# wuer5/OMGSR

Measured on AMD Instinct MI355X. Metric: SR images/sec, higher is better.
Workload: dtype fp16; 1 GPU; OMGSR-S 256->1024, batch=4/GPU, accurate tier (fp32 stream, fp16 MFMA operands + split corrections), tiled VAE 256/64; global_batch=4, latent_tile=64, tile_overlap=32, world_size=1, parallelism=dp1, weights=seeded random, SD2.1-base shapes

## Files before the change

omgsr_amd/csrc/igemm.hip:

```cpp
#include "common.hip.h"
#include "../../include/omgsr_hip.h"
#include "timing.hip.h"
#include "igemm_epilogue.hip.h"
#include "igemm_launch.hip.h"
#include <stdlib.h>
#include <stdio.h>
#include <string.h>

namespace omgsr { static int g_batch_invariant = 0; }
extern "C" int omgsr_set_batch_invariant(int on) { omgsr::g_batch_invariant = (on != 0); return 0; }

namespace {

omgsr_igemm_args policy_view(const omgsr_igemm_args& a) {
    omgsr_igemm_args p = a;
    if (omgsr::g_batch_invariant && a.batch == 1) {
        const int64_t howo = (int64_t)a.Ho * a.Wo;
        const int64_t rows = a.sample_rows > 0 ? a.sample_rows : howo;
        if (rows >= howo) p.N = (int32_t)(rows / howo);
        else { p.N = 1; p.Ho = 1; p.Wo = (int32_t)rows; }
        if (p.N < 1) p.N = 1;
    }
    return p;
}
// ... 369 lines not shown
    }
    if (a.workspace && splitk_plan(a, M64) > 1) return;
    if (omgsr::g_batch_invariant) return;
    const int howo = a.Ho * a.Wo;
    if (howo % 32) return;
    *nslot = howo / 32;
    *entries = (pow2 && gsz <= 32) ? a.gn_groups : a.Cout;
}
}

namespace {
bool gn_fusable(const omgsr_igemm_args& a_in) {
    static const char* off = getenv("OMGSR_GN_FUSE");
    if (off && off[0] == '0') return false;
    omgsr_igemm_args a = a_in;
    a.gn_scale_shift = nullptr;
    if (!omgsr::igemm_halo_gn_geometry_ok(a) || a.out_layout != OMGSR_LAYOUT_NHWC || a.act == OMGSR_ACT_GEGLU) return false;
    if ((int64_t)a.H * a.W * a.Cin >= (1ll << 31)) return false;
    if (a.workspace && splitk_plan(a, (int64_t)a.N * a.Ho * a.Wo) > 1) return false;
    if (!use_halo(a) || use_halo_phase(a)) return false;
    if (omgsr::igemm_halo_flat(a) != 0) return false;
    static const char* mc = getenv("OMGSR_GN_FUSE_MAX_COUT");
    static const int max_cout = mc ? atoi(mc) : 128;
    const int logical_cols = (a.act == OMGSR_ACT_GEGLU) ? 2 * a.Cout : a.Cout;
    return logical_cols <= max_cout;
}
}

extern "C" int32_t omgsr_igemm_gn_fusable(const omgsr_igemm_args* ap) { return (ap && gn_fusable(*ap)) ? 1 : 0; }
extern "C" int32_t omgsr_igemm_out_mx6_ok(const omgsr_igemm_args* ap) {
    if (!ap) return 0;
    omgsr_igemm_args a = *ap;
    a.out_mx = 6;
    return out_mx6_ok(a) ? 1 : 0;
}

extern "C" int32_t omgsr_igemm_gn_slots(const omgsr_igemm_args* ap) {
    if (!ap) return 0;
    int nslot, entries;
    gn_plan(*ap, &nslot, &entries);
    return nslot;
}

extern "C" int32_t omgsr_igemm_gn_entries(const omgsr_igemm_args* ap) {
    if (!ap) return 0;
    int nslot, entries;
    gn_plan(*ap, &nslot, &entries);
    return entries;
}

extern "C" int64_t omgsr_igemm_workspace_bytes(const omgsr_igemm_args* ap) {
    if (!ap || ap->mxf8) return 0;
    const int64_t M64 = (int64_t)ap->N * ap->Ho * ap->Wo;
    const int splits = splitk_plan(*ap, M64);
    if (splits < 2) return 0;
    const int logical_cols = (ap->act == OMGSR_ACT_GEGLU) ? 2 * ap->Cout : ap->Cout;
    return (int64_t)splits * M64 * (((logical_cols + 127) / 128) * 128) * 4;
}

namespace {
int validate_args(omgsr_igemm_args& a) {
    if (!a.in || !a.weight || !a.out) return OMGSR_E_BADARG;
    if (a.N <= 0 || a.H <= 0 || a.W <= 0 || a.Cin <= 0 || a.Cout <= 0 || a.Ho <= 0 || a.Wo <= 0 ||
        a.R <= 0 || a.S <= 0 || a.stride <= 0 || a.batch <= 0) return OMGSR_E_BADARG;
    if ((a.Cin & 7) || (a.Cout_pad & 127) || (a.K_pad % BK) || a.K_pad < a.R * a.S * a.Cin) return OMGSR_E_SHAPE;
    if (a.upsample != 0 && a.upsample != 1) return OMGSR_E_BADARG;
    const int64_t M64 = (int64_t)a.N * a.Ho * a.Wo;
    if (M64 >= (1ll << 31)) return OMGSR_E_SHAPE;
    const int logical_cols = (a.act == OMGSR_ACT_GEGLU) ? 2 * a.Cout : a.Cout;
    if (logical_cols > a.Cout_pad) return OMGSR_E_SHAPE;
    if (a.act == OMGSR_ACT_GEGLU && ((a.Cout & 31) || a.out_layout != OMGSR_LAYOUT_NHWC)) return OMGSR_E_SHAPE;
    if (a.out_layout == OMGSR_LAYOUT_T && (a.t_rows <= 0 || a.t_ld < a.t_rows || a.residual)) return OMGSR_E_BADARG;
    if (a.out_ld != 0 && (a.out_ld < a.Cout || a.out_layout != OMGSR_LAYOUT_NHWC)) return OMGSR_E_BADARG;
    if (a.res_el != OMGSR_EL_16 && a.res_el != OMGSR_EL_F32) return OMGSR_E_BADARG;
    if (a.res_el == OMGSR_EL_F32 && a.residual && a.act == OMGSR_ACT_GEGLU) return OMGSR_E_SHAPE;
    if (a.out_lo_off < 0) return OMGSR_E_BADARG;
    if (a.out_lo_off && (a.out_dtype != OMGSR_OUT_BF16 || a.out_layout != OMGSR_LAYOUT_NHWC || (a.Cout & 7) || (a.out_ld & 7) || (a.out_lo_off & 7) ||
                         a.out_lo_off < a.Cout || a.out_ld < a.out_lo_off + a.Cout || a.gn_partial)) return OMGSR_E_SHAPE;
    if (a.in_split && ((a.in_ld > 0 ? a.in_ld : a.Cin) & 15)) return OMGSR_E_SHAPE;
    if (a.in_ld < 0 || (a.in_ld & 7) || (a.in_ld > 0 && (a.in_ld > a.Cin || a.Cin > 2 * a.in_ld))) return OMGSR_E_SHAPE;
    if (a.in_ld == a.Cin) a.in_ld = 0;
    const int ksegs = 1 + (a.in_split ? 1 : 0) + (a.w_split ? 1 : 0);
    if (a.Cin % (8 * ksegs)) return OMGSR_E_SHAPE;
    if (a.mx_chunks16 < 0 || (a.mx_chunks16 > 0 && !mx_geometry_ok(a) && !omgsr::igemm_gmx_ok(a))) return OMGSR_E_SHAPE;
    if (a.mx_chunks16 > 0 && a.mx_fmt != 0 && a.mx_fmt != 8 && (a.mx_fmt != 6 || !mx_geometry_ok(a))) return OMGSR_E_SHAPE;
    if (a.out_mx != 0 && a.out_mx != 1 && a.out_mx != 6) return OMGSR_E_BADARG;
    if (a.out_mx == 6 && !out_mx6_ok(a)) return OMGSR_E_SHAPE;
    if (a.out_mx && (a.out_dtype != OMGSR_OUT_BF16 || a.out_layout != OMGSR_LAYOUT_NHWC || (a.Cout & 63) || a.out_lo_off || a.out_ld || a.gn_partial ||
                     omgsr::compute_dtype() != 1)) return OMGSR_E_SHAPE;
    if (a.gn_scale_shift && (a.gn_nimg <= 0 || a.gn_act != OMGSR_ACT_SILU || !gn_fusable(a))) return OMGSR_E_SHAPE;
    if (a.mxf8 != 0 && a.mxf8 != 1) return OMGSR_E_BADARG;
    if (a.mxf8 && !omgsr::mxfp8_gemm_ok(a)) return OMGSR_E_SHAPE;
    if (a.gn_partial) {
        int nslot, entries;
        gn_plan(a, &nslot, &entries);
        if (nslot <= 0 || a.gn_entries != entries) return OMGSR_E_BADARG;
    }
    return 0;
}

void work_of(const omgsr_igemm_args& a, double* flops, double* bytes, const bool out8 = false) {
    const int64_t M64 = (int64_t)a.N * a.Ho * a.Wo;
    const int logical_cols = (a.act == OMGSR_ACT_GEGLU) ? 2 * a.Cout : a.Cout;
    const int ksegs = 1 + (a.in_split ? 1 : 0) + (a.w_split ? 1 : 0);
    *flops = 2.0 * (double)M64 * (double)a.R * a.S * (a.Cin / ksegs) * (double)logical_cols * a.batch;
    const double out_b = out8 ? 1.0 + 1.0 / 32.0 : (a.out_dtype == OMGSR_OUT_F32 ? 4.0 : (a.out_lo_off ? 4.0 : 2.0)), res_b = a.residual ? (a.res_el == OMGSR_EL_F32 ? 4.0 : 2.0) : 0.0;
    const double eb = a.mxf8 ? 1.0 + 1.0 / 32.0 : 2.0;
    *bytes = (eb * ((double)a.N * a.H * a.W * (a.in_ld > 0 ? a.in_ld : a.Cin) + (double)a.Cout_pad * a.K_pad) + (double)M64 * a.Cout * (out_b + res_b)) * a.batch;
}

Geo geo_of(const omgsr_igemm_args& a) {
    Geo g{};
    g.M = (int)((int64_t)a.N * a.Ho * a.Wo);
    g.HoWo = a.Ho * a.Wo;
    g.Hv = a.H << a.upsample;
    g.Wv = a.W << a.upsample;
    g.nk = a.K_pad / BK;
    g.splits = 1; g.nk_total = g.nk;
    return g;
}
}

extern "C" int omgsr_igemm_multi_plan(omgsr_igemm_args* args, int32_t count) {
    if (!args || count <= 0) return OMGSR_E_BADARG;
    static const char* off = getenv("OMGSR_MULTI");
    int total = 0, total_ph = 0, total_flat = 0;
    bool all_flat_ok = true;
    for (int i = 0; i < count; ++i) {
        args[i].group_tiles = 0;
        total += omgsr::igemm_halo_tiles_form(args[i], 0);
        total_ph += omgsr::igemm_halo_tiles(args[i], true);
        const int tf = omgsr::igemm_halo_tiles_form(args[i], 1);
        all_flat_ok = all_flat_ok && tf > 0;
        total_flat += tf > 0 ? tf : 0;
    }
    if ((off && off[0] == '0') || omgsr::g_batch_invariant) return 0;
    const bool flat = all_flat_ok && total_flat < total;
    for (int i = 0; i < count; ++i) args[i].group_tiles = (args[i].upsample && args[i].weight_ph) ? total_ph : (flat ? -total_flat : total);
    return 0;
}

extern "C" int omgsr_igemm_multi(const omgsr_igemm_args* args, int32_t count, void* stream) {
    if (!args || count <= 0) return OMGSR_E_BADARG;
    hipStream_t st = (hipStream_t)stream;
    constexpr int MAXG = 8;
    omgsr_igemm_args grp[MAXG];
    Geo geo[MAXG];
    int ng = 0, mode = -1;
    double gf = 0.0, gb = 0.0;
    long long gm = 0;
    auto flush = [&]() -> int {
        if (ng == 0) return 0;
        int rc;
        {
            const int logical_cols = (grp[0].act == OMGSR_ACT_GEGLU) ? 2 * grp[0].Cout : grp[0].Cout;
            omgsr::TimingScope ts(OMGSR_TK_IGEMM, gf, gb, st, gm, logical_cols, (long long)grp[0].R * grp[0].S * grp[0].Cin);
            ts.rec.variant = ng == 1 ? (mode == 1 ? 6 : 3) : (mode == 1 ? 8 : 7);
            if (grp[0].gn_scale_shift) ts.rec.variant = ng == 1 ? 10 : 11;
            if (grp[0].mx_chunks16 > 0 && grp[0].mx_fmt == 6) ts.rec.variant = mode == 1 ? (ng == 1 ? 16 : 17) : (ng == 1 ? 13 : 14);
            rc = ng == 1 ? omgsr::igemm_halo_launch(grp[0], geo[0], st, mode == 1) : omgsr::igemm_halo_launch_multi(grp, geo, ng, st, mode == 1);
        }
        ng = 0; gf = gb = 0.0; gm = 0;
        return rc;
    };
    for (int i = 0; i < count; ++i) {
        omgsr_igemm_args a = args[i];
// ... 366 lines not shown
```

omgsr_amd/csrc/igemm_halo_body.hip.h:

```cpp
#pragma once
#include "common.hip.h"
#include "../../include/omgsr_hip.h"
#include "igemm_epilogue.hip.h"
#include "igemm_launch.hip.h"
#include <stdlib.h>
#include <type_traits>

namespace {

constexpr int TH = 8, TW = 32;
template <int TAPS, bool BIG = false> struct HaloGeo {
    static constexpr int KS = TAPS == 9 ? 3 : 2;
    static constexpr int PW = TW + KS - 1, PH = TH + KS - 1, PROWS = PH * PW;
    static constexpr int APIECES = BIG ? 27 : (PROWS + 15) / 16, APW = (APIECES + 3) / 4;
    static constexpr int A_BYTES = APIECES * 1024;
    static constexpr int NB = TAPS == 9 ? 3 : 4;
    static constexpr int DUMMY_OFF = 2 * A_BYTES, B_OFF = DUMMY_OFF + 2048;
    static constexpr int LDS_BYTES = B_OFF + NB * 128 * 64;
};
constexpr int BN = 128, B_BYTES = BN * 64, BPW = 2;
constexpr int LDS_BYTES = HaloGeo<9>::LDS_BYTES > HaloGeo<4>::LDS_BYTES ? HaloGeo<9>::LDS_BYTES : HaloGeo<4>::LDS_BYTES;
static_assert(HaloGeo<9>::APIECES == 22 && HaloGeo<9>::APW == 6 && HaloGeo<4>::APIECES == 19 && HaloGeo<4>::APW == 5, "piece counts");
constexpr int LDS_BYTES_BIG = HaloGeo<9, true>::LDS_BYTES;
constexpr int GN_MAX_CIN = 1024, LDS_BYTES_GN = HaloGeo<9>::LDS_BYTES + GN_MAX_CIN * 8;
// ... 272 lines not shown
#pragma unroll
                for (int j = 0; j < FN; ++j)
                    asm volatile("s_nop 3\n\tv_mfma_scale_f32_32x32x64_f8f6f4 %0, %1, %2, %0, %3, %4 op_sel_hi:[0,0,0]"
                                 : "+v"(acc[i][j]) : "v"(b8[j]), "v"(a8[i]), "v"(sw), "v"(sa));
                if constexpr (LATE) {
                    if (i == FM / 2 - 1) {
                        __builtin_amdgcn_sched_barrier(0);
                        issue_dma();
                        __builtin_amdgcn_sched_barrier(0);
                    }
                }
            }
            return;
        }
        x8_t<T> af[2][FM], bf[2][FN];
#pragma unroll
        for (int i = 0; i < FM; ++i) {
            af[0][i] = *reinterpret_cast<const x8_t<T>*>(As + i * AIMM + aoff[tap][FLAT ? 0 : i]);
            af[1][i] = *reinterpret_cast<const x8_t<T>*>(As + i * AIMM + (aoff[tap][FLAT ? 0 : i] ^ 32));
        }
#pragma unroll
        for (int j = 0; j < FN; ++j) {
            bf[0][j] = *reinterpret_cast<const x8_t<T>*>(Bs + j * 32 * 64 + boff0);
            bf[1][j] = *reinterpret_cast<const x8_t<T>*>(Bs + j * 32 * 64 + boff1);
        }
        if constexpr (PRIO) __builtin_amdgcn_s_setprio(1);
#pragma unroll
        for (int ks = 0; ks < 2; ++ks) {
#pragma unroll
            for (int i = 0; i < FM; ++i)
#pragma unroll
                for (int j = 0; j < FN; ++j) acc[i][j] = mfma32(bf[ks][j], af[ks][i], acc[i][j]);
            if constexpr (LATE) {
                if (ks == 0) {
                    __builtin_amdgcn_sched_barrier(0);
                    issue_dma();
                    __builtin_amdgcn_sched_barrier(0);
                }
            }
        }
        if constexpr (GNF != 0 && tap >= 2 && tap < 2 + APW) {
            if (cc + 1 < ncc) {
                __builtin_amdgcn_sched_barrier(0);
                u32x4_t g_raw;
                f32x4_t g_tb[4];
                gn_read(tap - 2, par ^ 1, cc + 1, g_raw, g_tb);
                *gn_slot(tap - 2, par ^ 1) = gn_math(tap - 2, g_raw, g_tb);
            }
        }
        if constexpr (PRIO) __builtin_amdgcn_s_setprio(0);
    };
    auto chunk = [&](auto par_c, auto f8_c, const int cc) {
        const int s0 = cc * TAPS;
        step(std::integral_constant<int, 0>{}, par_c, f8_c, cc, s0 + 0);
        step(std::integral_constant<int, 1>{}, par_c, f8_c, cc, s0 + 1);
        step(std::integral_constant<int, 2>{}, par_c, f8_c, cc, s0 + 2);
        step(std::integral_constant<int, 3>{}, par_c, f8_c, cc, s0 + 3);
        if constexpr (TAPS == 9) {
            step(std::integral_constant<int, 4>{}, par_c, f8_c, cc, s0 + 4);
            step(std::integral_constant<int, 5>{}, par_c, f8_c, cc, s0 + 5);
            step(std::integral_constant<int, 6>{}, par_c, f8_c, cc, s0 + 6);
            step(std::integral_constant<int, 7>{}, par_c, f8_c, cc, s0 + 7);
            step(std::integral_constant<int, 8>{}, par_c, f8_c, cc, s0 + 8);
        }
    };
    if (g.main_prio == 1) __builtin_amdgcn_s_setprio(1);
    else if (g.main_prio == 2) __builtin_amdgcn_s_setprio(2);
    int cc = cbeg;
    const int e16 = (SPLITK && n16 > ncc) ? ncc : n16;
    for (; cc < e16; cc += 2) {
        chunk(std::integral_constant<int, 0>{}, std::integral_constant<int, 0>{}, cc);
        if (cc + 1 < e16) chunk(std::integral_constant<int, 1>{}, std::integral_constant<int, 0>{}, cc + 1);
    }
    if constexpr (MX && std::is_same<T, f16_t>::value && !NARROW && ABL == 0 && !PRIO) {
        asm volatile("s_nop 7\n\ts_nop 7" ::: "memory");
        for (; cc < ncc; cc += 2) {
            chunk(std::integral_constant<int, 0>{}, std::integral_constant<int, 1>{}, cc);
            if (cc + 1 < ncc) chunk(std::integral_constant<int, 1>{}, std::integral_constant<int, 1>{}, cc + 1);
        }
        asm volatile("s_nop 15\n\ts_nop 15\n\ts_nop 15\n\ts_nop 15\n\ts_nop 15\n\ts_nop 15" ::: "memory");
    }

    if (g.main_prio) __builtin_amdgcn_s_setprio(0);
    int mb[FM], nv[FM];
    int colsv = (PHASE ? p.W : p.Wo) - x0; colsv = colsv > TW ? TW : colsv;
#pragma unroll
    for (int i = 0; i < FM; ++i) {
        const int y = y0 + FM * wm + i;
        mb[i] = PHASE ? (img * p.Ho + 2 * y + ph_a) * p.Wo + 2 * x0 + ph_b : (img * p.Ho + y) * p.Wo + x0;
        nv[i] = (y < (PHASE ? p.H : p.Ho)) ? colsv : 0;
        if (FP) {
            mb[i] = f0 + TW * (FM * wm + i);
            const int left = p.Ho * FP - mb[i];
            nv[i] = left < 0 ? 0 : (left > TW ? TW : left);
        }
    }
    if constexpr (ABL == 1) { if (p.alpha != 12345.0f) return; }
    {
        float* epi = reinterpret_cast<float*>(lds) + wave * 32 * (WTN + 4);
        const int64_t slot = PHASE ? ((int64_t)(img * per_img + trem) * 2 + wm) * 4 + bidy : (int64_t)(img * per_img + trem) * 2 + wm;
        float* gn_dst = (p.gn_partial && !NARROW) ? p.gn_partial + slot * p.gn_entries * 2 : nullptr;
        igemm_epilogue<T, WTN, FM, FN, OUT6>(p, acc, epi, lane, mb, nv, n0 + wn * WTN, 0, gn_dst, 0, PHASE ? 2 : (FP ? -FP : 1), FP ? img * p.Ho * p.Wo : 0);
    }
}

OMGSR_DEVINL bool phase_block_map(const int b, const int T, const int n8, const bool chunked, int& tile, int& phase) {
    constexpr int CH = 64;
    const int xcd = b & 7, idx = b >> 3;
    int base, cnt;
    if (n8 > 0) { cnt = n8 >> 3; base = xcd * cnt; }
    else {
        const int q = T >> 3, r = T & 7;
        base = xcd < r ? xcd * (q + 1) : r * (q + 1) + (xcd - r) * q;
        cnt = xcd < r ? q + 1 : q;
    }
    if (idx >= 4 * cnt) return false;
    if (chunked) {
        const int chunk = idx / (4 * CH), r = idx - chunk * 4 * CH;
        const int left = cnt - chunk * CH, sz = left < CH ? left : CH;
        phase = r / sz;
        tile = base + chunk * CH + (r - phase * sz);
    } else {
        tile = base + (idx >> 2); phase = idx & 3;
    }
    return tile < T;
}

template <typename T, int ABL, bool PRIO, bool NARROW = false, int TAPS = 9, int MX = 0, int FLAT = 0, int GNF = 0, bool OUT6 = false>
__global__ __launch_bounds__(256, 2) void igemm_halo_kernel(const omgsr_igemm_args p, const IgemmGeo g) {
    int tile, phase;
    if (TAPS == 4 && g.interleave) {
        if (!phase_block_map((int)blockIdx.x, g.ntm * g.ntn, 0, g.interleave == 2, tile, phase)) return;
    } else {
        tile = xcd_remap((int)blockIdx.x, g.ntm * g.ntn); phase = (int)blockIdx.y;
    }
    halo_body<T, ABL, PRIO, NARROW, TAPS, MX, FLAT, GNF, false, OUT6>(p, g, tile, phase);
}

constexpr int HALO_MULTI_MAX = 8;
struct HaloMulti {
    omgsr_igemm_args p[HALO_MULTI_MAX];
    IgemmGeo g[HALO_MULTI_MAX];
    int start[HALO_MULTI_MAX + 1];
    int count;
};
template <typename T, bool NARROW, int TAPS, int MX = 0, int FLAT = 0, int GNF = 0, bool SPLITK = false, bool OUT6 = false>
__global__ __launch_bounds__(256, 2) void igemm_halo_multi_kernel(const HaloMulti m) {
    int s = 0, tile, phase;
    if (TAPS == 4 && m.g[0].interleave) {
        while (s + 1 < m.count && (int)blockIdx.x >= 4 * m.start[s + 1]) ++s;
        if (!phase_block_map((int)blockIdx.x - 4 * m.start[s], m.g[s].ntm * m.g[s].ntn, m.start[s + 1] - m.start[s], m.g[0].interleave == 2, tile, phase)) return;
    } else {
        while (s + 1 < m.count && (int)blockIdx.x >= m.start[s + 1]) ++s;
        const int bid = (int)blockIdx.x - m.start[s];
        if (bid >= m.g[s].ntm * m.g[s].ntn) return;
        tile = xcd_remap(bid, m.g[s].ntm * m.g[s].ntn); phase = (int)blockIdx.y;
    }
    halo_body<T, 0, false, NARROW, TAPS, MX, FLAT, GNF, SPLITK, OUT6>(m.p[s], m.g[s], tile, phase);
}


static inline int halo_flat_eligible(const omgsr_igemm_args& a) {
    static const char* off = getenv("OMGSR_HALO_FLAT");
    if (off && off[0] == '0') return 0;
    if (a.gn_scale_shift) return 0;
    if (a.out_mx == 6) return 0;
    static const char* mw = getenv("OMGSR_HALO_FLAT_MAXW");
    static const int maxw = mw ? atoi(mw) : 80;
    const int logical_cols = (a.act == OMGSR_ACT_GEGLU) ? 2 * a.Cout : a.Cout;
    const int64_t ldo = a.out_ld > 0 ? a.out_ld : a.Cout;
    if (a.R != 3 || a.S != 3 || a.stride != 1 || a.upsample || a.Wo != a.W || a.Ho != a.H || a.Wo > maxw || a.Wo < 4 || logical_cols < 96 || (a.Cout & 7) || (ldo & 7) ||
        a.out_layout != OMGSR_LAYOUT_NHWC || a.act == OMGSR_ACT_GEGLU) return 0;
    return a.Wo + 2;
}
static inline int halo_flat_tiles_per_image(const omgsr_igemm_args& a) { return (a.Ho * (a.Wo + 2) + TH * TW - 1) / (TH * TW); }
static inline int halo_grid_tiles_per_image(const omgsr_igemm_args& a) { return ((a.Wo + TW - 1) / TW) * ((a.Ho + TH - 1) / TH); }
static inline int halo_flat_pitch(const omgsr_igemm_args& a) {
    const int P = halo_flat_eligible(a);
    if (!P) return 0;
    if (a.group_tiles < 0) return P;
    if (a.group_tiles > 0) return 0;
    return halo_flat_tiles_per_image(a) < halo_grid_tiles_per_image(a) ? P : 0;
}

static inline bool halo_geo(const omgsr_igemm_args& a, IgemmGeo& g, const bool phase) {
    const int logical_cols = (a.act == OMGSR_ACT_GEGLU) ? 2 * a.Cout : a.Cout;
    static const char* mp = getenv("OMGSR_HALO_MAINPRIO");
    g.main_prio = mp ? atoi(mp) : 0;
    static const char* il = getenv("OMGSR_PHASE_INTERLEAVE");
    g.interleave = phase ? (il ? atoi(il) : 2) : 0;
    g.nk = a.Cin / 32;
    g.tiles_x = ((phase ? a.W : a.Wo) + TW - 1) / TW;
    g.tiles_y = ((phase ? a.H : a.Ho) + TH - 1) / TH;
    g.flat = phase ? 0 : halo_flat_pitch(a);
    if (g.flat) { g.tiles_x = (a.Ho * g.flat + TH * TW - 1) / (TH * TW); g.tiles_y = 1; }
    g.ntm = a.N * g.tiles_x * g.tiles_y;
    const bool narrow = logical_cols <= 32 && !phase;
    g.ntn = narrow ? 1 : (logical_cols + BN - 1) / BN;
    return narrow;
}

constexpr bool COLS_128 = false, COLS_32 = true;
constexpr int MX_NONE = 0, MX_FP8 = 1, MX_FP6 = 6;
constexpr int FLAT_OFF = 0, FLAT_22 = 1, FLAT_27 = 2;
constexpr int GNF_OFF = 0, GNF_ON = 1;
constexpr bool OUT6_ON = true, SPLITK_ON = true;
constexpr int FLAT_22_MAX_PITCH = 47;

template <typename T, bool NARROW, int TAPS, int MX = MX_NONE, int FLAT = FLAT_OFF, int GNF = GNF_OFF, bool OUT6 = false>
constexpr auto halo_one = &igemm_halo_kernel<T, 0, false, NARROW, TAPS, MX, FLAT, GNF, OUT6>;
template <typename T, bool NARROW, int TAPS, int MX = MX_NONE, int FLAT = FLAT_OFF, int GNF = GNF_OFF, bool OUT6 = false>
constexpr auto halo_group = &igemm_halo_multi_kernel<T, NARROW, TAPS, MX, FLAT, GNF, false, OUT6>;
constexpr int halo_lds_bytes(const int flat, const int gnf) { return gnf ? LDS_BYTES_GN : flat == FLAT_27 ? LDS_BYTES_BIG : LDS_BYTES; }

static inline dim3 halo_grid(const IgemmGeo& g, const bool phase) {
    return (phase && g.interleave) ? dim3(32 * ((g.ntm * g.ntn + 7) / 8)) : dim3(g.ntm * g.ntn, phase ? 4 : 1, 1);
}
static inline dim3 halo_multi_grid(const IgemmGeo& g0, const unsigned blocks, const bool phase) {
    return (phase && g0.interleave) ? dim3(4 * blocks) : dim3(blocks, phase ? 4 : 1, 1);
}

struct HaloPack { int blocks; bool narrow, flat; };
static inline HaloPack halo_multi_pack(const omgsr_igemm_args* a, const IgemmGeo* g0, const int count, const bool phase, HaloMulti& m) {
    HaloPack k{0, false, false};
    m.count = count;
    for (int i = 0; i < count; ++i) {
        m.p[i] = a[i];
        m.g[i] = g0[i];
        const bool narrow = halo_geo(a[i], m.g[i], phase);
        k.narrow = k.narrow || narrow;
        k.flat = k.flat || m.g[i].flat != 0;
        m.start[i] = k.blocks;
        k.blocks += (m.g[i].ntm * m.g[i].ntn + 7) & ~7;
    }
    m.start[count] = k.blocks;
    return k;
}

struct HaloJob {
    const omgsr_igemm_args* a; const IgemmGeo* g;
    const HaloMulti* m; unsigned blocks;
    hipStream_t st;
};
static inline HaloJob halo_job(const omgsr_igemm_args& a, const IgemmGeo& g, hipStream_t st) { return HaloJob{&a, &g, nullptr, 0u, st}; }
static inline HaloJob halo_job(const void* halo_multi, const unsigned blocks, hipStream_t st) {
    return HaloJob{nullptr, nullptr, reinterpret_cast<const HaloMulti*>(halo_multi), blocks, st};
}
template <typename T, bool NARROW, int TAPS, int MX = MX_NONE, int FLAT = FLAT_OFF, int GNF = GNF_OFF, bool OUT6 = false>
int halo_run(const HaloJob& j) {
    constexpr int lds = halo_lds_bytes(FLAT, GNF);
    if (j.m) return launch_lds<halo_group<T, NARROW, TAPS, MX, FLAT, GNF, OUT6>>(halo_multi_grid(j.m->g[0], j.blocks, TAPS == 4), dim3(256), lds, j.st, *j.m);
    return launch_lds<halo_one<T, NARROW, TAPS, MX, FLAT, GNF, OUT6>>(halo_grid(*j.g, TAPS == 4), dim3(256), lds, j.st, *j.a, *j.g);
}
template <int MX>
int halo_mx_run(const HaloJob& j, const bool phase, const bool splitk) {
    if (phase) return halo_run<f16_t, COLS_128, 4, MX>(j);
    if (splitk && !j.m) return OMGSR_E_BADARG;
    if (splitk) return launch_lds<igemm_halo_multi_kernel<f16_t, COLS_128, 9, MX, FLAT_OFF, GNF_OFF, SPLITK_ON>>(halo_multi_grid(j.m->g[0], j.blocks, false), dim3(256), LDS_BYTES, j.st, *j.m);
    return halo_run<f16_t, COLS_128, 9, MX>(j);
}

}
```

omgsr_amd/ops.py:

```python
from __future__ import annotations

import ctypes as C
import os
from contextlib import contextmanager
from dataclasses import dataclass
from typing import NamedTuple, Optional

import torch

from . import _lib
from ._lib import AttnArgs, IgemmArgs, check

ACT_NONE, ACT_SILU, ACT_GELU_TANH, ACT_GEGLU = 0, 1, 2, 3
OUT_STREAM, OUT_BF16, OUT_F32 = -1, 0, 1
LAYOUT_NHWC, LAYOUT_T = 0, 1
EL_16, EL_F32, EL_SPLIT, EL_MX, EL_MX6, EL_MXFP8 = 0, 1, 2, 3, 4, 5
MX_LO_SHIFT = 11


def _el_of_split(split: int) -> int:
    return {1: EL_16, 2: EL_SPLIT, 3: EL_MX, 4: EL_MX6}[split]


_ACT = torch.bfloat16
# ... 151 lines not shown
        raise _lib.OmgsrError(f"{name}: tensor is on {t.device}; the OMGSR HIP path runs on an MI355X only")
    if not t.is_contiguous():
        raise ValueError(f"{name}: must be contiguous")
    return t


def _round_up(x: int, m: int) -> int:
    return (x + m - 1) // m * m


class _GemmGroup:

    def __init__(self):
        self.blocks, self.whats, self.keep = [], [], []

    def add(self, a: "IgemmArgs", what: str, keep=()) -> None:
        self.blocks.append(a)
        self.whats.append(what)
        self.keep.append(tuple(keep))

    def launch(self) -> None:
        n = len(self.blocks)
        if n == 0:
            return
        lib = _lib.load()
        arr = (IgemmArgs * n)(*self.blocks)
        if lib.omgsr_igemm_mxfp8_multi_ok(arr, n):
            check(lib.omgsr_igemm_mxfp8_multi(arr, n, _stream()), "omgsr_igemm_mxfp8_multi(" + ", ".join(self.whats) + ")")
        else:
            for a, what in zip(self.blocks, self.whats):
                check(lib.omgsr_igemm(C.byref(a), _stream()), what)
        self.keep.clear()


_GEMM_GROUP: Optional[_GemmGroup] = None


@contextmanager
def gemm_group():
    global _GEMM_GROUP
    if _GEMM_GROUP is not None:
        raise RuntimeError("ops.gemm_group: scopes do not nest")
    grp = _GEMM_GROUP = _GemmGroup()
    try:
        yield grp
    except BaseException:
        _GEMM_GROUP = None
        raise
    _GEMM_GROUP = None
    grp.launch()


def _igemm(a: "IgemmArgs", device, what: str, z_batched_api: bool = False, workspace: bool = True, keep=()) -> None:
    if _GEMM_GROUP is not None and a.mxf8 == 1:
        _GEMM_GROUP.add(a, what, keep)
        return
    lib = _lib.load()
    need = 0 if (not workspace or (z_batched_api and _BATCH_INVARIANT)) else lib.omgsr_igemm_workspace_bytes(C.byref(a))
    ws = None
    if need > 0:
        ws = torch.empty(need // 4, device=device, dtype=torch.float32)
        a.workspace = ws.data_ptr()
    check(lib.omgsr_igemm(C.byref(a), _stream()), what)



@dataclass
class PackedWeight:
    w: torch.Tensor
    bias: Optional[torch.Tensor]
    cout: int
    cin: int
    R: int
    S: int
    geglu: bool = False
    w_cm: Optional[torch.Tensor] = None
    split: int = 1
    mx: Optional[tuple] = None
    mx_fmt: int = 0
    w_split: int = 1
    in_ld: int = 0
    w_ph: Optional[torch.Tensor] = None
    w_scale: Optional[torch.Tensor] = None

    @property
    def fp8(self) -> bool:
        return self.w_scale is not None

    @property
    def cout_pad(self) -> int:
        return self.w.shape[0]

    @property
    def k_pad(self) -> int:
        return self.w.shape[1]

    @property
    def row_channels(self) -> int:
        return self.in_ld or self.cin


def _segments(w: torch.Tensor, split: int, w_split: int) -> torch.Tensor:
    w_hi = w.to(act_dtype()).float()
    segs = [w_hi] * split
    if w_split == 2:
        segs.append((w - w_hi).to(act_dtype()).float())
    return torch.cat(segs, dim=-1) if len(segs) > 1 else w_hi


def _mx_rows(w: torch.Tensor, s1: int, s2: int) -> torch.Tensor:
    w_hi = w.to(torch.float16)
    hi8 = (w_hi.float() * 2.0 ** s1).clamp(-448.0, 448.0).to(torch.float8_e4m3fn).view(torch.uint8)
    lo8 = ((w - w_hi.float()) * 2.0 ** s2).clamp(-448.0, 448.0).to(torch.float8_e4m3fn).view(torch.uint8)
    return torch.cat([w_hi.contiguous().view(torch.uint8).reshape(*w.shape[:-1], 2 * w.shape[-1]), hi8, lo8], dim=-1)


def _e2m3_blocks(v: torch.Tensor) -> torch.Tensor:
    lead, Cc = v.shape[:-1], v.shape[-1]
    b = v.reshape(-1, Cc // 32, 32).float()
    m = b.abs().amax(-1)
    sb = ((m.view(torch.int32) >> 23) - 2).clamp(min=0)
    inv = ((254 - sb) << 23).to(torch.int32).view(torch.float32).unsqueeze(-1)
    s_ = b * inv
    a = s_.abs().clamp(max=7.5)
    eb = (a.view(torch.int32) >> 23).clamp(min=127)
    q = torch.round(a * ((257 - eb) << 23).to(torch.int32).view(torch.float32)).to(torch.int64)
    code = (q + ((eb.to(torch.int64) - 127) << 3)) | (((s_.view(torch.int32).to(torch.int64) >> 26) & 32))
    c4 = code.reshape(*code.shape[:-1], 8, 4)
    v24 = c4[..., 0] | (c4[..., 1] << 6) | (c4[..., 2] << 12) | (c4[..., 3] << 18)
    string = torch.stack([v24 & 0xFF, (v24 >> 8) & 0xFF, (v24 >> 16) & 0xFF], dim=-1).to(torch.uint8).reshape(*code.shape[:-1], 24)
    R, nb = string.shape[0], string.shape[1]
    out = torch.zeros((R, nb // 2, 64), dtype=torch.uint8, device=v.device)
    st = string.reshape(R, nb // 2, 2, 24)
    sbv = sb.reshape(R, nb // 2, 2).to(torch.uint8)
    for h in (0, 1):
        out[..., 16 * h:16 * h + 16] = st[..., h, :16]
        out[..., 32 + 16 * h:40 + 16 * h] = st[..., h, 16:]
        out[..., 40 + 16 * h] = sbv[..., h]
    return out.reshape(*lead, Cc)


def _mx6_rows(w: torch.Tensor) -> torch.Tensor:
    w_hi = w.to(torch.float16)
    return torch.cat([w_hi.contiguous().view(torch.uint8).reshape(*w.shape[:-1], 2 * w.shape[-1]), _e2m3_blocks(w_hi.float()), _e2m3_blocks(w - w_hi.float())], dim=-1)


def _mx_shift(t: torch.Tensor) -> int:
    import math
    m = float(t.abs().max())
    return max(-100, min(100, 7 - math.floor(math.log2(m)))) if m > 0 else 0


def _pack_mx(w: torch.Tensor, bias, cout: int, cin: int, R: int, S: int, dev, upsample_phases: bool = False, fmt: int = 8) -> "PackedWeight":
    if fmt == 6 and (R, S) != (3, 3):
        raise ValueError("the fp6 form (split 4) serves the 3x3 stride-1 convolutions of the halo-tile kernel")
    rows = (lambda t: _mx6_rows(t)) if fmt == 6 else (lambda t: _mx_rows(t, s1, s2))
    if (R, S) not in ((3, 3), (1, 1)) or cin % 64 or act_dtype() != torch.float16:
        raise ValueError("the mixed-precision (MX) form serves 3x3 and 1x1 convolutions (linears) with Cin % 64 == 0 in the fp16 compute type")
    ph = _phase_kernels(w) if upsample_phases else None
    both = w if ph is None else torch.cat([w.reshape(-1), ph.reshape(-1)])
    both_hi = both.to(torch.float16).float()
    s1, s2 = _mx_shift(both_hi), _mx_shift(both - both_hi)
    kslots = 2 * cin
    cout_pad = _round_up(cout, 256 if cout >= 256 else 128)
    out = torch.zeros((cout_pad, R * S * kslots), device=dev, dtype=torch.float16)
    out[:cout] = rows(w).reshape(cout, R * S * 4 * cin).contiguous().view(torch.float16)
    w_cm = out.view(cout_pad, 9, kslots // 32, 32).permute(2, 1, 0, 3).contiguous() if R == 3 else None
    w_ph = None
    if ph is not None:
        full = torch.zeros((4, cout_pad, 4 * kslots), device=dev, dtype=torch.float16)
        full[:, :cout] = rows(ph).reshape(4, cout, 4 * 4 * cin).contiguous().view(torch.float16)
        w_ph = full.view(4, cout_pad, 4, kslots // 32, 32).permute(0, 3, 2, 1, 4).contiguous()
    b = None if bias is None else bias.detach().to(device=dev, dtype=torch.float32).contiguous()
    if fmt == 6:
        return PackedWeight(out, b, cout, kslots, R, S, w_cm=w_cm, split=4, w_split=1, in_ld=kslots, w_ph=w_ph, mx=(cin // 32, 127, 127, 127, 127), mx_fmt=6)
    return PackedWeight(out, b, cout, kslots, R, S, w_cm=w_cm, split=3, w_split=1, in_ld=kslots, w_ph=w_ph,
                        mx=(cin // 32, 127 - s1, 127 - MX_LO_SHIFT, 127 - s2, 127))


def _phase_kernels(w: torch.Tensor) -> torch.Tensor:
    rows = {0: ([0], [1, 2]), 1: ([0, 1], [2])}
    w64 = w.double()
    out = []
    for a in (0, 1):
        for b in (0, 1):
            k = torch.zeros((w.shape[0], 2, 2, w.shape[3]), dtype=torch.float64, device=w.device)
            for dy, rs in enumerate(rows[a]):
                for dx, ss in enumerate(rows[b]):
                    for r in rs:
                        for s_ in ss:
                            k[:, dy, dx] += w64[:, r, s_]
            out.append(k.float())
    return torch.stack(out, 0)


def pack_conv_weight(weight: torch.Tensor, bias: Optional[torch.Tensor], device=None, cout_multiple: int = 1,
                     split: int = 1, w_split: int = 1, upsample_phases: bool = False) -> PackedWeight:
    cout, cin, R, S = weight.shape
    dev = device or weight.device
    if cout % cout_multiple:
        extra = _round_up(cout, cout_multiple) - cout
        weight = torch.cat([weight.detach().to(dev), torch.zeros((extra, cin, R, S), device=dev, dtype=weight.dtype)], dim=0)
        if bias is not None:
            bias = torch.cat([bias.detach().to(dev), torch.zeros(extra, device=dev, dtype=bias.dtype)], dim=0)
        cout += extra
    cin8 = _round_up(cin, 8)
    w = _note_weight_range(weight.detach().to(device=dev, dtype=torch.float32)).permute(0, 2, 3, 1)
    if cin8 != cin:
        w = torch.nn.functional.pad(w, (0, cin8 - cin))
    if split in (3, 4):
        if cin8 != cin:
            raise ValueError("the mixed-precision (MX) form needs Cin % 64 == 0")
        return _pack_mx(w, bias if bias is None else bias.detach().to(dev), cout, cin, R, S, dev, upsample_phases, fmt=6 if split == 4 else 8)
    if split not in (1, 2) or w_split not in (1, 2):
        raise ValueError("split / w_split must be 1 or 2")
    if w_split == 2 and bool(torch.equal(w.to(act_dtype()).float(), w)):
        ph_exact = True
        if upsample_phases and R == 3 and S == 3:
            ph0 = _phase_kernels(w)
            ph_exact = bool(torch.equal(ph0.to(act_dtype()).float(), ph0))
        if ph_exact:
            w_split = 1
    in_ld = cin8 * split
    w_raw = w
    w = _segments(w, split, w_split)
    cin8 = w.shape[-1]
    w = w.reshape(cout, R * S * cin8)
    k_pad = _round_up(w.shape[1], 32)
    cout_pad = _round_up(cout, 256 if cout >= 256 else 128)
    out = torch.zeros(cout_pad, k_pad, device=dev, dtype=act_dtype())
    out[:cout, : w.shape[1]] = w.to(act_dtype())
    b = None if bias is None else bias.detach().to(device=dev, dtype=torch.float32).contiguous()
    w_cm = None
    if R == 3 and S == 3 and cin8 % 32 == 0:
        w_cm = out.view(cout_pad, 9, cin8 // 32, 32).permute(2, 1, 0, 3).contiguous()
    w_ph = None
    if upsample_phases and w_cm is not None and in_ld % 32 == 0:
        ph = _segments(_phase_kernels(w_raw), split, w_split).reshape(4, cout, 4 * cin8)
        full = torch.zeros((4, cout_pad, 4 * cin8), device=dev, dtype=act_dtype())
        full[:, :cout] = ph.to(act_dtype())
        w_ph = full.view(4, cout_pad, 4, cin8 // 32, 32).permute(0, 3, 2, 1, 4).contiguous()
    return PackedWeight(out, b, cout, cin8, R, S, w_cm=w_cm, split=split, w_split=w_split, in_ld=in_ld, w_ph=w_ph)


def pack_linear_weight(weight: torch.Tensor, bias: Optional[torch.Tensor], device=None, split: int = 1, w_split: int = 1) -> PackedWeight:
    return pack_conv_weight(weight[:, :, None, None], bias, device, split=split, w_split=w_split)


def pack_geglu_weight(weight: torch.Tensor, bias: Optional[torch.Tensor], device=None, split: int = 1, w_split: int = 1) -> PackedWeight:
    two_inner, cin = weight.shape
    inner = two_inner // 2
    if inner % 32:
        raise ValueError("GEGLU inner dim must be a multiple of 32")
    a, g = weight[:inner], weight[inner:]
    w = torch.stack([a.reshape(inner // 32, 32, cin), g.reshape(inner // 32, 32, cin)], dim=1).reshape(two_inner, cin)
    pw = pack_linear_weight(w, None, device, split=split, w_split=w_split)
    if bias is not None:
        ba, bg = bias[:inner], bias[inner:]
        b = torch.stack([ba.reshape(-1, 32), bg.reshape(-1, 32)], dim=1).reshape(two_inner)
        pw.bias = b.detach().to(device=pw.w.device, dtype=torch.float32).contiguous()
    pw.cout = inner
    pw.geglu = True
    return pw



@dataclass
class Mxfp8:
    codes: torch.Tensor
    scales: torch.Tensor

    @property
    def shape(self):
        return self.codes.shape

    def reshape(self, *lead) -> "Mxfp8":
        lead = lead[:-1] if lead and lead[-1] == -1 else lead
        return Mxfp8(self.codes.reshape(*lead, self.codes.shape[-1]), self.scales.reshape(*lead, self.scales.shape[-1]))


def _mxfp8_like(x: torch.Tensor) -> Mxfp8:
    return Mxfp8(torch.empty(x.shape, device=x.device, dtype=torch.uint8),
                 torch.empty((*x.shape[:-1], x.shape[-1] // 32), device=x.device, dtype=torch.uint8))


def parse_fp8_fused_quant(value: Optional[str]) -> dict:
    if value is None or value.strip() == "":
        return dict(FP8_FUSED_QUANT_DEFAULT)
    if value.strip() not in ("0", "1"):
        raise ValueError(f"OMGSR_FP8_FUSED_QUANT must be 0 or 1, got {value!r}")
    on = value.strip() == "1"
    return {"layernorm": on, "gemm": on}


FP8_FUSED_QUANT_DEFAULT = {"layernorm": True, "gemm": True}
FP8_FUSED_QUANT = parse_fp8_fused_quant(os.environ.get("OMGSR_FP8_FUSED_QUANT"))


def _row_pitch(x: torch.Tensor, name: str) -> int:
    K = x.shape[-1]
    if x.dim() < 2 or x.is_contiguous():
        return K
    ld = x.stride(-2)
    ok = x.stride(-1) == 1 and ld >= K and all(x.stride(i) == x.stride(i + 1) * x.shape[i + 1] for i in range(x.dim() - 2))
    if not ok:
        raise ValueError(f"{name}: expected a dense tensor or a column window of one")
    return ld


def quantize_mxfp8(x: torch.Tensor, out: Optional[Mxfp8] = None, out_col: Optional[int] = None) -> Mxfp8:
    if x.dtype not in (torch.bfloat16, torch.float32):
        raise TypeError(f"quantize_mxfp8: expected bfloat16 or float32, got {x.dtype}")
    K = x.shape[-1]
    if K % 128:
        raise ValueError(f"quantize_mxfp8: K = {K} is not a multiple of 128")
    rows = x.numel() // K
    el = EL_F32 if x.dtype == torch.float32 else EL_16
    if out_col is not None:
        if out is None:
            raise ValueError("quantize_mxfp8: out_col needs `out`")
        Kw = out.codes.shape[-1]
        if (out.codes.shape[:-1] != x.shape[:-1] or out.scales.shape != (*x.shape[:-1], Kw // 32) or Kw % 128 or out_col % 128 or out_col < 0
                or out_col + K > Kw or not (out.codes.is_contiguous() and out.scales.is_contiguous())):
            raise ValueError("quantize_mxfp8: x does not fit `out` at out_col")
        check(_lib.load().omgsr_quantize_mxfp8_ld(x.data_ptr(), el, rows, K, _row_pitch(x, "quantize_mxfp8"), out.codes.data_ptr() + out_col,
# ... 39 lines not shown
def _fill_mxfp8(a: IgemmArgs, codes_ptr: int, scales_ptr: int, pw: PackedWeight) -> None:
    a.in_, a.in_scale = codes_ptr, scales_ptr
    a.weight, a.w_scale, a.bias = pw.w.data_ptr(), pw.w_scale.data_ptr(), _ptr(pw.bias)
    a.mxf8 = 1
    a.Cin, a.Cout, a.Cout_pad, a.K_pad = pw.cin, pw.cout, pw.cout_pad, pw.k_pad
    _fill_taps_1x1(a)


def pack_conv_weight_mxfp8(weight: torch.Tensor, bias: Optional[torch.Tensor], device=None) -> PackedWeight:
    if _PRECISE or _ACT != torch.bfloat16:
        raise ValueError("an fp8 (MXFP8) layer needs the bf16 compute type (the fp8 tier); the accurate tier and fp16 have none")
    dev = device or weight.device
    cout, cin, R, S = weight.shape
    if (R, S) != (3, 3) or cin % 128:
        raise ValueError(f"an fp8 (MXFP8) conv needs a 3x3 kernel and in_channels % 128 == 0, got {tuple(weight.shape)}")
    cout8 = _round_up(cout, 8)
    cout_pad = _round_up(cout8, 128)
    w = torch.zeros((cout_pad, 9, cin), device=dev, dtype=torch.bfloat16)
    w[:cout] = weight.detach().to(device=dev, dtype=torch.bfloat16).permute(0, 2, 3, 1).reshape(cout, 9, cin)
    q = quantize_mxfp8(w)
    codes = q.codes.view(cout_pad, 9, cin // 64, 64).permute(2, 1, 0, 3).contiguous()
    sc = torch.zeros((cin // 64, cout_pad, 2, 16), device=dev, dtype=torch.uint8)
    sc[..., :9] = q.scales.view(cout_pad, 9, cin // 64, 2).permute(2, 0, 3, 1)
    b = None
    if bias is not None:
        b = torch.zeros(cout8, device=dev, dtype=torch.float32)
        b[:cout] = bias.detach().to(device=dev, dtype=torch.float32)
    return PackedWeight(codes.view(cin // 64 * 9 * cout_pad, 64), b, cout8, cin, 3, 3, w_cm=codes, w_scale=sc)


def pack_conv_weight_mxfp8_up(weight: torch.Tensor, bias: Optional[torch.Tensor], device=None) -> PackedWeight:
    if _PRECISE or _ACT != torch.bfloat16:
        raise ValueError("an fp8 (MXFP8) layer needs the bf16 compute type (the fp8 tier); the accurate tier and fp16 have none")
    dev = device or weight.device
    cout, cin, R, S = weight.shape
    if (R, S) != (3, 3) or cin % 128:
        raise ValueError(f"an fp8 (MXFP8) up-sampling conv needs a 3x3 kernel and in_channels % 128 == 0, got {tuple(weight.shape)}")
    cout8 = _round_up(cout, 8)
    cout_pad = _round_up(cout8, 128)
    ph = _phase_kernels(weight.detach().to(device=dev, dtype=torch.bfloat16).permute(0, 2, 3, 1).float())
    w = torch.zeros((4, cout_pad, 4, cin), device=dev, dtype=torch.float32)
    w[:, :cout] = ph.reshape(4, cout, 4, cin)
    q = quantize_mxfp8(w)
    codes = q.codes.view(4, cout_pad, 4, cin // 64, 64).permute(0, 3, 2, 1, 4).contiguous()
    sc = q.scales.view(4, cout_pad, 4, cin // 64, 2).permute(0, 3, 1, 4, 2).contiguous()
    b = None
    if bias is not None:
        b = torch.zeros(cout8, device=dev, dtype=torch.float32)
        b[:cout] = bias.detach().to(device=dev, dtype=torch.float32)
    return PackedWeight(codes.view(-1, 64), b, cout8, cin, 3, 3, w_ph=codes, w_scale=sc)



def to_operand(x: torch.Tensor, split: int = 1) -> torch.Tensor:
    if x.dtype == _ACT:
        if split != 1:
            raise ValueError("to_operand: a 16-bit tensor cannot be split (split operands exist in the accurate tier only)")
        return x
    _req(x, torch.float32, "x")
    Cc = x.shape[-1]
    y = torch.empty((*x.shape[:-1], min(split, 2) * Cc), device=x.device, dtype=_ACT)
    check(_lib.load().omgsr_to_operand(x.data_ptr(), y.data_ptr(), x.numel() // Cc, Cc, _el_of_split(split), _ovf(x.device),
                                       _stream()), "omgsr_to_operand")
    return y


def _out_tensor(shape, cout: int, out_dtype: int, out_split: int, device) -> torch.Tensor:
    if out_dtype == OUT_STREAM:
        out_dtype = OUT_F32 if _PRECISE else OUT_BF16
        if out_split != 1:
            raise ValueError("out_split applies to operand outputs (out_dtype=OUT_BF16)")
    if out_dtype == OUT_F32:
        return torch.empty((*shape, cout), device=device, dtype=torch.float32)
    return torch.empty((*shape, cout * min(out_split, 2)), device=device, dtype=_ACT)



def _fill_weight(a: IgemmArgs, pw: PackedWeight, x_ptr: int, scales_ptr: Optional[int] = None) -> None:
    a.in_, a.weight, a.bias, a.weight_cm = x_ptr, pw.w.data_ptr(), _ptr(pw.bias), _ptr(pw.w_cm)
    a.Cin, a.Cout, a.Cout_pad, a.K_pad = pw.cin, pw.cout, pw.cout_pad, pw.k_pad
    a.overflow_flag = _ovf(pw.w.device)
    a.in_ld = pw.row_channels if pw.row_channels != pw.cin else 0
    a.in_split = int(pw.split >= 2)
    a.w_split = int(pw.w_split == 2)
    if pw.mx is not None:
        a.mx_chunks16, a.mx_scale_w1, a.mx_scale_a1, a.mx_scale_w2, a.mx_scale_a2 = pw.mx
        a.mx_fmt = pw.mx_fmt
    if scales_ptr is not None:
        _fill_mxfp8(a, x_ptr, scales_ptr, pw)


def _fill_taps_1x1(a: IgemmArgs) -> None:
    a.R, a.S, a.stride, a.pad_top, a.pad_left, a.upsample = 1, 1, 1, 0, 0, 0


def _fill_gemm(a: IgemmArgs, M: int, batch: int = 1, in_bstride: int = 0, w_bstride: int = 0, out_bstride: int = 0) -> None:
    a.N, a.H, a.W, a.Ho, a.Wo = 1, 1, M, 1, M
    _fill_taps_1x1(a)
    a.batch, a.in_bstride, a.w_bstride, a.out_bstride = batch, in_bstride, w_bstride, out_bstride


def _fill_out(a: IgemmArgs, out: torch.Tensor, out_split: int, residual: Optional[torch.Tensor], cout: int) -> None:
    a.out = out.data_ptr()
    a.out_dtype = OUT_F32 if out.dtype == torch.float32 else OUT_BF16
    a.out_lo_off = cout if out_split == 2 else 0
    a.out_ld = out.shape[-1] if out_split == 2 else 0
    a.out_mx = {3: 1, 4: 6}.get(out_split, 0)
    if residual is not None:
        a.residual, a.res_el = residual.data_ptr(), _el(residual, "residual")


def _fill_out_slice(a: IgemmArgs, buf: torch.Tensor, first: int, *, ld: int = 0, lo_off: int = 0, t_rows: Optional[int] = None) -> None:
    a.out, a.out_dtype = buf.data_ptr() + 2 * first, OUT_BF16
    a.out_ld, a.out_lo_off = ld, lo_off
    if t_rows is not None:
        a.out_layout, a.t_rows, a.t_ld = LAYOUT_T, t_rows, buf.shape[-1]


def _fill_out_mxfp8(a: IgemmArgs, dst: Mxfp8, row0: int, col0: int) -> tuple:
    Kw = dst.codes.shape[-1]
    a.out, a.out_dtype, a.out_ld = dst.codes.data_ptr() + row0 * Kw + col0, OUT_BF16, Kw
    return dst.scales.data_ptr() + row0 * (Kw // 32) + col0 // 32, Kw // 32


def _igemm_out_mxfp8(a: IgemmArgs, scale: tuple, what: str) -> None:
    check(_lib.load().omgsr_igemm_out_mxfp8(C.byref(a), scale[0], scale[1], _stream()), what)


def _out_mxfp8_dst(what: str, out_mxfp8, pw: PackedWeight, lead, device, col0: int = 0, *, residual=None, gate=None, plain: bool = True) -> Optional[Mxfp8]:
    if out_mxfp8 is None or out_mxfp8 is False:
        return None
    if not pw.fp8:
        raise ValueError(f"{what}: out_mxfp8 needs an fp8-packed weight (the MXFP8 GEMM's epilogue writes the form)")
    if residual is not None or gate is not None or not plain:
        raise ValueError(f"{what}: out_mxfp8 goes with bias and act only (no residual, gate, GroupNorm statistics, split or fp32 output)")
    if pw.cout % 32:
        raise ValueError(f"{what}: out_mxfp8 needs Cout % 32 == 0, got {pw.cout}")
    if out_mxfp8 is True:
        if col0:
            raise ValueError(f"{what}: out_mxfp8=True writes a dense result")
        if pw.cout % 128:
            raise ValueError(f"{what}: a dense Mxfp8 result needs Cout % 128 == 0, got {pw.cout}")
        return Mxfp8(torch.empty((*lead, pw.cout), device=device, dtype=torch.uint8), torch.empty((*lead, pw.cout // 32), device=device, dtype=torch.uint8))
    if not isinstance(out_mxfp8, Mxfp8):
        raise TypeError(f"{what}: out_mxfp8 is True or an Mxfp8")
    Kw = out_mxfp8.codes.shape[-1]
    if (tuple(out_mxfp8.codes.shape[:-1]) != tuple(lead) or tuple(out_mxfp8.scales.shape) != (*lead, Kw // 32) or Kw % 128 or col0 % 128 or col0 < 0
            or col0 + pw.cout > Kw or not (out_mxfp8.codes.is_contiguous() and out_mxfp8.scales.is_contiguous())):
        raise ValueError(f"{what}: the result does not fit the Mxfp8 destination at column {col0}")
    return out_mxfp8


def _conv_args(a: IgemmArgs, x: torch.Tensor, pw: PackedWeight, stride, pad, upsample, act, residual, gate, out_dtype, alpha, out, out_split,
               sample_rows):
    if x.dtype == torch.float32:
        x = to_operand(x, pw.split)
    _req(x, act_dtype(), "x")
    N, H, W, Cin = x.shape
    if Cin != pw.row_channels:
        raise ValueError(f"conv2d: input has {Cin} channels, packed weight expects {pw.row_channels}")
    if isinstance(pad, int):
        pad = (pad, pad, pad, pad)
    pt, pb, pl, pr = pad
    Hv, Wv = (H * 2, W * 2) if upsample else (H, W)
    Ho = (Hv + pt + pb - pw.R) // stride + 1
    Wo = (Wv + pl + pr - pw.S) // stride + 1
    if pw.geglu:
# ... 1078 lines not shown
```

Before: 21.39 images/s.

## Fold weight-split low part into spare output columns for narrow 3x3 convs

```diff
diff --git a/omgsr_amd/csrc/igemm.hip b/omgsr_amd/csrc/igemm.hip
--- a/omgsr_amd/csrc/igemm.hip
+++ b/omgsr_amd/csrc/igemm.hip
@@ -475,6 +475,9 @@
     if (a.in_ld == a.Cin) a.in_ld = 0;
     const int ksegs = 1 + (a.in_split ? 1 : 0) + (a.w_split ? 1 : 0);
     if (a.Cin % (8 * ksegs)) return OMGSR_E_SHAPE;
+    if (a.w_split < 0 || a.w_split > 2) return OMGSR_E_BADARG;
+    if (a.w_split == 2 && (!a.in_split || a.in_ld <= 0 || 2 * a.Cin != 3 * a.in_ld || (a.in_ld % 32) || a.Cout > 16 || a.R != 3 || a.S != 3 || !a.weight_cm ||
+                           a.mx_chunks16 > 0 || a.act == OMGSR_ACT_GEGLU)) return OMGSR_E_SHAPE;
     if (a.mx_chunks16 < 0 || (a.mx_chunks16 > 0 && !mx_geometry_ok(a) && !omgsr::igemm_gmx_ok(a))) return OMGSR_E_SHAPE;
     if (a.mx_chunks16 > 0 && a.mx_fmt != 0 && a.mx_fmt != 8 && (a.mx_fmt != 6 || !mx_geometry_ok(a))) return OMGSR_E_SHAPE;
     if (a.out_mx != 0 && a.out_mx != 1 && a.out_mx != 6) return OMGSR_E_BADARG;
diff --git a/omgsr_amd/csrc/igemm_halo_body.hip.h b/omgsr_amd/csrc/igemm_halo_body.hip.h
--- a/omgsr_amd/csrc/igemm_halo_body.hip.h
+++ b/omgsr_amd/csrc/igemm_halo_body.hip.h
@@ -378,6 +378,18 @@
     }
 
     if (g.main_prio) __builtin_amdgcn_s_setprio(0);
+    if constexpr (NARROW) {
+        if (p.w_split == 2) {
+            const bool c16 = p.Cout > 8;
+#pragma unroll
+            for (int i = 0; i < FM; ++i)
+#pragma unroll
+                for (int r = 0; r < 8; ++r) {
+                    const float part = c16 ? acc[i][0][r + 8] : (r < 4 ? acc[i][0][r + 4] : 0.0f);
+                    acc[i][0][r] += part;
+                }
+        }
+    }
     int mb[FM], nv[FM];
     int colsv = (PHASE ? p.W : p.Wo) - x0; colsv = colsv > TW ? TW : colsv;
 #pragma unroll
@@ -492,6 +504,7 @@
     if (g.flat) { g.tiles_x = (a.Ho * g.flat + TH * TW - 1) / (TH * TW); g.tiles_y = 1; }
     g.ntm = a.N * g.tiles_x * g.tiles_y;
     const bool narrow = logical_cols <= 32 && !phase;
+    if (narrow && a.w_split == 2) g.nk = a.in_ld / 32;
     g.ntn = narrow ? 1 : (logical_cols + BN - 1) / BN;
     return narrow;
 }
diff --git a/omgsr_amd/ops.py b/omgsr_amd/ops.py
--- a/omgsr_amd/ops.py
+++ b/omgsr_amd/ops.py
@@ -257,6 +257,7 @@
     in_ld: int = 0
     w_ph: Optional[torch.Tensor] = None
     w_scale: Optional[torch.Tensor] = None
+    cm_spare: bool = False
 
     @property
     def fp8(self) -> bool:
@@ -367,6 +368,17 @@
                             k[:, dy, dx] += w64[:, r, s_]
             out.append(k.float())
     return torch.stack(out, 0)
+
+
+def _spare_column_cm(w: torch.Tensor, cout_pad: int) -> torch.Tensor:
+    cout, cin8 = w.shape[0], w.shape[-1]
+    c8 = _round_up(cout, 8)
+    w_hi = w.to(act_dtype()).float()
+    w_lo = (w - w_hi).to(act_dtype()).float()
+    rows = torch.zeros((cout_pad, 9, 2 * cin8), device=w.device, dtype=torch.float32)
+    rows[:cout] = torch.cat([w_hi, w_hi], dim=-1).reshape(cout, 9, 2 * cin8)
+    rows[c8:c8 + cout, :, :cin8] = w_lo.reshape(cout, 9, cin8)
+    return rows.to(act_dtype()).view(cout_pad, 9, 2 * cin8 // 32, 32).permute(2, 1, 0, 3).contiguous()
 
 
 def pack_conv_weight(weight: torch.Tensor, bias: Optional[torch.Tensor], device=None, cout_multiple: int = 1,
@@ -409,13 +421,17 @@
     w_cm = None
     if R == 3 and S == 3 and cin8 % 32 == 0:
         w_cm = out.view(cout_pad, 9, cin8 // 32, 32).permute(2, 1, 0, 3).contiguous()
+    cm_spare = (w_cm is not None and split == 2 and w_split == 2 and _round_up(cout, 8) <= 16 and in_ld % 32 == 0
+                and os.environ.get("OMGSR_NARROW_SPARE", "1") != "0")
+    if cm_spare:
+        w_cm = _spare_column_cm(w_raw, cout_pad)
     w_ph = None
     if upsample_phases and w_cm is not None and in_ld % 32 == 0:
         ph = _segments(_phase_kernels(w_raw), split, w_split).reshape(4, cout, 4 * cin8)
         full = torch.zeros((4, cout_pad, 4 * cin8), device=dev, dtype=act_dtype())
         full[:, :cout] = ph.to(act_dtype())
         w_ph = full.view(4, cout_pad, 4, cin8 // 32, 32).permute(0, 3, 2, 1, 4).contiguous()
-    return PackedWeight(out, b, cout, cin8, R, S, w_cm=w_cm, split=split, w_split=w_split, in_ld=in_ld, w_ph=w_ph)
+    return PackedWeight(out, b, cout, cin8, R, S, w_cm=w_cm, split=split, w_split=w_split, in_ld=in_ld, w_ph=w_ph, cm_spare=cm_spare)
 
 
 def pack_linear_weight(weight: torch.Tensor, bias: Optional[torch.Tensor], device=None, split: int = 1, w_split: int = 1) -> PackedWeight:
@@ -621,7 +637,7 @@
     a.overflow_flag = _ovf(pw.w.device)
     a.in_ld = pw.row_channels if pw.row_channels != pw.cin else 0
     a.in_split = int(pw.split >= 2)
-    a.w_split = int(pw.w_split == 2)
+    a.w_split = 2 if pw.cm_spare else int(pw.w_split == 2)
     if pw.mx is not None:
         a.mx_chunks16, a.mx_scale_w1, a.mx_scale_a1, a.mx_scale_w2, a.mx_scale_a2 = pw.mx
         a.mx_fmt = pw.mx_fmt
```

After: 21.48 images/s (median of 5 runs). About the same (+0.4%).
